# XuZhang1211/PVPUFormer

Hardware: AMD Instinct MI355X
Metric: 448x448 images/sec fwd+bwd, ViT-B VPUFormer (higher is better)
Workload: dtype bf16

## Files before the change

include/vpu_hip.h:

```cpp
#ifndef VPU_HIP_H
#define VPU_HIP_H
#include <stdint.h>

#ifdef __cplusplus
extern "C" {
#endif

#define VPU_BF16 0
#define VPU_F32 1

#define VPU_EPI_BIAS 1
#define VPU_EPI_PREACT 2
#define VPU_EPI_GELU 4
#define VPU_EPI_RELU 8
#define VPU_EPI_DGELU 16
#define VPU_EPI_DRELU 32
#define VPU_EPI_RESID 64
#define VPU_EPI_AFFINE 128
#define VPU_EPI_ACCUM 256
#define VPU_EPI_OUT_F32 512
#define VPU_EPI_SAVE_DGELU 1024
#define VPU_EPI_MULAUX 2048

typedef struct vpu_gemm_desc {
// ... 141 lines not shown
int vpu_click_keys_batched(const vpu_eval_obj* objs, int32_t n, uint8_t* err, int32_t* scratch, float* dist, int32_t Hm,
                           int32_t Wm, int32_t max_hw, void* stream);
typedef struct vpu_box_row {
    const float* prev;
    const uint8_t* gt;
    const uint8_t* valid;
    int32_t H, W, r0, r1, c0, c1, mirror, n_obj;
} vpu_box_row;
int vpu_box_prompts_batched(const vpu_box_row* rows, int32_t n_rows, const float* points, int32_t n_batch, int32_t S_h,
                            int32_t S_w, float pred_thresh, uint8_t* masks, int32_t* counts, int32_t* roots, int32_t* slots,
                            int32_t* table, int32_t kmax, int32_t* boxes, int32_t* flag, void* stream);
int vpu_cc_roots(const uint8_t* mask, int32_t* roots, int32_t B, int32_t H, int32_t W, void* stream);
int vpu_cc_table(const int32_t* roots, int32_t* slots, int32_t* table, int32_t kmax, int32_t B, int32_t H, int32_t W,
                 void* stream);

int vpu_disk_maps(const float* points, const int32_t* boxes, float* out, int32_t B, int32_t n, int32_t H, int32_t W,
                  float radius, void* stream);

int vpu_patch_im2col(const float* image4, const float* disks, void* cols, int32_t B, int32_t H, int32_t W, int32_t P,
                     int32_t win_tokens, int32_t dtype, void* stream);
int vpu_patch_im2col_prenorm(const float* image4, const float* disks, void* cols, int32_t B, int32_t H, int32_t W, int32_t P,
                             int32_t win_tokens, int32_t dtype, void* stream);
int vpu_patch_im2col_floor(const float* image4, const float* disks, void* cols, int32_t B, int32_t H, int32_t W, int32_t P,
                           int32_t wside, int32_t prenorm, int32_t dtype, void* stream);
int vpu_window_permute(const void* x, void* y, int32_t B, int32_t g, int32_t wg, int32_t C, int32_t dir, int32_t dtype,
                       void* stream);

int vpu_pixel_shuffle2(const void* in, void* out, const float* bias, int32_t B, int32_t h, int32_t w, int32_t C,
                       int32_t dir, int32_t dtype, void* stream);
int vpu_space_to_depth2_crop(const void* in, void* out, int32_t B, int32_t g, int32_t C, int32_t dir, int32_t dtype,
                             void* stream);
int vpu_pixel_shuffle2_gn_stats(const void* in, void* out, const float* bias, double* stats, int32_t B, int32_t h, int32_t w,
                                int32_t C, int32_t dtype, void* stream);
int vpu_groupnorm_apply(const void* x, const float* w, const float* b, void* y, float* mean, float* rstd, const double* stats,
                        int32_t B, int64_t HW, int32_t C, float eps, int32_t gelu, int32_t dtype, void* stream);
int vpu_pixel_unshuffle2_nblk(int32_t C);
int vpu_pixel_unshuffle2_sums(const void* in, void* out, float* part, int32_t B, int32_t h, int32_t w, int32_t C,
                              int32_t dtype, void* stream);
int vpu_groupnorm_nchunk(void);
int vpu_groupnorm_fwd(const void* x, const float* w, const float* b, void* y, float* mean, float* rstd, double* stats,
                      int32_t B, int64_t HW, int32_t C, float eps, int32_t gelu, int32_t dtype, void* stream);
int vpu_groupnorm_bwd(const void* dy, const void* x, const float* w, const float* b, const float* mean,
                      const float* rstd, void* dx, float* part, double* stats, int32_t B, int64_t HW, int32_t C,
                      int32_t gelu, int32_t dtype, void* stream);
int vpu_bilinear_cl_fwd(const void* in, int32_t ld_in, void* out, int32_t ld_out, int32_t B, int32_t h, int32_t w,
                        int32_t H, int32_t W, int32_t C, int32_t dtype, void* stream);
int vpu_bilinear_cl_bwd(const void* dout, int32_t ld_out, void* din, int32_t ld_in, int32_t B, int32_t h, int32_t w,
                        int32_t H, int32_t W, int32_t C, int32_t dtype, void* stream);
int vpu_upsum_relu(void* io, const void* const* z, const int32_t* h, const int32_t* w, int32_t n, int32_t B, int32_t H,
                   int32_t W, int32_t C, int32_t dtype, void* stream);
int vpu_head_grad_fused(const void* dfn, const void* y, const float* inv, const float* dout, const void* x, const float* w,
                        const float* mask, void* dx, float* part, float* part_b, int64_t rows, int64_t HW, int32_t C,
                        int32_t dtype, void* stream);
int vpu_gate_stats(const void* Q, const void* Kt, float* cg, int32_t* argq, float* sg, int32_t* argc, int32_t B,
                   int32_t nq, int32_t N, int32_t C, int32_t dtype, void* stream);
int vpu_gate_apply(const void* x, const float* cg, const float* sg, void* out, int32_t B, int32_t N, int32_t C,
                   int32_t dtype, void* stream);
int vpu_gate_bwd(const void* dout, const void* x, const float* cg, const int32_t* argq, const float* sg,
                 const int32_t* argc, void* dx, int32_t accum, void* dQ, void* dK, float* part, int32_t B, int32_t nq,
                 int32_t N, int32_t C, int32_t dtype, void* stream);
int vpu_gate_fwd_n(const void* const* Q, const void* const* K, const void* x, void* const* out, float* cg, int32_t* argq,
                   float* sg, int32_t* argc, int32_t n, int32_t B, int32_t nq, int32_t N, int32_t C, int32_t dtype, void* stream);
int vpu_gate_bwd_n(const void* const* dout, const void* x, const float* cg, const int32_t* argq, const float* sg,
                   const int32_t* argc, void* dx, int32_t accum, void* const* dQ, void* const* dK, float* part, int32_t n,
                   int32_t B, int32_t nq, int32_t N, int32_t C, int32_t dtype, void* stream);
int vpu_convseg_fwd(const void* x, const float* w, const float* bias, const float* mask, float* out, int64_t rows,
                    int64_t HW, int32_t C, int32_t dtype, void* stream);
int vpu_convseg_bwd_nblk(int64_t rows);
int vpu_convseg_bwd(const float* dout, const void* x, const float* w, const float* mask, void* dx, int32_t accum,
                    float* part, float* part_b, int64_t rows, int64_t HW, int32_t C, int32_t dtype, void* stream);

int vpu_upsample_ac_fwd(const float* in, float* out, int64_t planes, int32_t h, int32_t w, int32_t H, int32_t W,
                        void* stream);
int vpu_upsample_ac_bwd(const float* dout, float* din, int64_t planes, int32_t h, int32_t w, int32_t H, int32_t W,
                        void* stream);
int vpu_p2cl_fwd_bwd(const float* prob, const float* gt, const int32_t* slot_mask_idx, const float* override_masks,
                     float* loss_part, float* dprob, float grad_scale, int32_t B, int32_t S, int32_t H, int32_t W,
                     void* stream);
int vpu_p2cl_up_nband(int32_t h, int32_t w);
int vpu_p2cl_up_fwd_bwd(const float* sim_low, const float* gt, const int32_t* slot_mask_idx, const float* override_masks,
                        float* loss_part, float* dsim_low, float grad_scale, int32_t B, int32_t S, int32_t h, int32_t w,
                        int32_t H, int32_t W, void* stream);
int vpu_nfl_dice_scratch_doubles(int32_t B);
int vpu_nfl_dice_fwd_bwd(const float* logits, const float* gt, double* sums, float* out, float* dlogits, float w_nfl,
                         float w_dice, int32_t B, int64_t HW, void* stream);

int vpu_loss_finalize(const float* out, const float* part, int32_t B, int32_t npart, double inv_count, float w_nfl,
                      float w_dice, float w_pcl, float iter_weight, float* res, void* stream);

int vpu_adam_step(float* p, const float* g, float* m, float* v, void* shadow_bf16, int64_t n, float lr, float beta1,
                  float beta2, float eps, float weight_decay, int32_t step, float grad_scale, void* stream);
int vpu_adam_step_groups(float* p, const float* g, float* m, float* v, void* shadow_bf16, int64_t n,
                         const int64_t* seg_end, const float* seg_lr, const float* seg_wd, int32_t nseg, float beta1,
                         float beta2, float eps, int32_t decoupled_wd, int32_t step, float grad_scale, void* stream);
int vpu_adam_step_hyper(float* p, const float* g, float* m, float* v, void* shadow_bf16, int64_t n, const float* hyper,
                        const int64_t* seg_end, const float* seg_scale, const float* seg_wd, int32_t nseg, float beta1,
                        float beta2, float eps, float weight_decay, int32_t decoupled_wd, void* stream);


#ifdef __cplusplus
}
#endif
#endif
```

pvpuformer_amd/_lib.py:

```python
import ctypes as C
import os

_HERE = os.path.dirname(os.path.abspath(__file__))
LIB_PATH = os.path.join(_HERE, os.environ.get("VPU_LIB_FILE") or
                        ("libvpu_hip_diag.so" if os.environ.get("VPU_LIB_DIAG", "0") == "1" else "libvpu_hip.so"))

BF16, F32 = 0, 1

EPI_BIAS, EPI_PREACT, EPI_GELU, EPI_RELU, EPI_DGELU, EPI_DRELU = 1, 2, 4, 8, 16, 32
EPI_RESID, EPI_AFFINE, EPI_ACCUM, EPI_OUT_F32 = 64, 128, 256, 512
EPI_SAVE_DGELU, EPI_MULAUX = 1024, 2048


class GemmDesc(C.Structure):
    _fields_ = [
        ("A", C.c_void_p), ("B", C.c_void_p), ("C", C.c_void_p), ("bias", C.c_void_p), ("resid", C.c_void_p),
        ("aux", C.c_void_p), ("preact", C.c_void_p),
        ("M", C.c_int32), ("N", C.c_int32), ("K", C.c_int32),
        ("lda", C.c_int32), ("ldb", C.c_int32), ("ldc", C.c_int32), ("ldr", C.c_int32), ("ldaux", C.c_int32),
        ("batch", C.c_int32), ("inner", C.c_int32),
        ("sAo", C.c_int64), ("sAi", C.c_int64), ("sBo", C.c_int64), ("sBi", C.c_int64),
        ("sCo", C.c_int64), ("sCi", C.c_int64), ("sRo", C.c_int64), ("sRi", C.c_int64),
        ("transA", C.c_int32), ("transB", C.c_int32), ("dtype", C.c_int32), ("flags", C.c_int32),
        ("resid_period", C.c_int32),
# ... 44 lines not shown
    "vpu_l2norm_fwd": [_P, _P, _P, _L, _I, _I, _P],
    "vpu_l2norm_bwd": [_P, _P, _P, _P, _L, _I, _I, _P],
    "vpu_attn_fwd": [_P, _P, _P, _P, _P, _I, _I, _I, _I, _I, _I, _F, _P],
    "vpu_attn_bwd": [_P, _P, _P, _P, _P, _P, _P, _P, _P, _P, _I, _I, _I, _I, _I, _I, _I, _F, _P],
    "vpu_xattn_fwd": [_P, _P, _P, _P, _P, _I, _I, _I, _I, _I, _I, _I, _I, _F, _P],
    "vpu_xattn_bwd": [_P, _P, _P, _P, _P, _P, _P, _P, _P, _P, _I, _I, _I, _I, _I, _I, _I, _I, _I, _I, _F, _P],
    "vpu_xattn_fwd_split": [_P, _P, _P, _P, _P, _I, _I, _I, _I, _I, _I, _I, _I, _F, _I, _I, _P],
    "vpu_xattn_bwd_split": [_P, _P, _P, _P, _P, _P, _P, _P, _P, _P, _I, _I, _I, _I, _I, _I, _I, _I, _I, _I, _F, _I, _I, _P],
    "vpu_attn_combine": [_P, _P, _P, _P, _I, _I, _I, _I, _I, _I, _I, _P],
    "vpu_sum_groups": [_P, _P, _L, _I, _L, _I, _P],
    "vpu_add_bcast": [_P, _P, _P, _L, _L, _I, _P],
    "vpu_add4": [_P, _P, _P, _P, _P, _L, _I, _P],
    "vpu_cast2d": [_P, _I, _L, _P, _I, _L, _L, _I, _I, _P],
    "vpu_cast2d_batched": [C.POINTER(CastJob), _I, _P],
    "vpu_fanout_add": [_P, C.POINTER(C.c_void_p), C.POINTER(C.c_int32), _I, _L, _I, _P],
    "vpu_dropout_mask": [_P, _I, _F, C.c_uint64, _P, _P],
    "vpu_fill_f32": [_P, _F, _L, _P],
    "vpu_fill_ranges_f32": [_P, C.POINTER(C.c_int64), C.POINTER(C.c_int64), _I, _F, _P],
    "vpu_debug_spin": [_P, _I, _L, _P],
    "vpu_debug_gemm_times": [_P],
    "vpu_sigmoid_to_channel": [_P, _P, _I, _L, _I, _I, _P],
    "vpu_act_bwd": [_P, _L, _P, _L, _P, _L, _L, _I, _I, _I, _P],
    "vpu_pue_encode": [_P, _P, _P, _P, _P, _I, _I, _I, _I, _I, _I, _P],
    "vpu_cc_roots": [_P, _P, _I, _I, _I, _P],
    "vpu_cc_table": [_P, _P, _P, _I, _I, _I, _I, _P],
    "vpu_edt": [_P, _P, _P, _I, _I, _I, _I, _P],
    "vpu_chamfer5": [_P, _P, _P, _I, _I, _I, _I, _P],
    "vpu_pue_scribble_rows": [_P, _P, _P, _P, _I, _I, _I, _I, _I, _I, _P],
    "vpu_draw_polyline": [_P, _P, _I, _I, _I, _I, _P],
    "vpu_mask_bbox": [_P, _F, _P, _I, _P, _I, _I, _I, _P],
    "vpu_masked_argmax": [_P, _P, _P, _I, _I, _I, _P],
    "vpu_error_masks": [_P, _P, _P, _P, _I, _I, _P],
    "vpu_roi_resize_batched": [_P, _I, _P, _I, _I, _I, _I, _P],
    "vpu_roi_paste_batched": [_P, _I, _P, _I, _I, _F, _F, _I, _P],
    "vpu_click_keys_batched": [_P, _I, _P, _P, _P, _I, _I, _I, _P],
    "vpu_box_prompts_batched": [_P, _I, _P, _I, _I, _I, _F, _P, _P, _P, _P, _P, _I, _P, _P, _P],
    "vpu_disk_maps": [_P, _P, _P, _I, _I, _I, _I, _F, _P],
    "vpu_patch_im2col": [_P, _P, _P, _I, _I, _I, _I, _I, _I, _P],
    "vpu_patch_im2col_prenorm": [_P, _P, _P, _I, _I, _I, _I, _I, _I, _P],
    "vpu_patch_im2col_floor": [_P, _P, _P, _I, _I, _I, _I, _I, _I, _I, _P],
    "vpu_window_permute": [_P, _P, _I, _I, _I, _I, _I, _I, _P],
    "vpu_space_to_depth2_crop": [_P, _P, _I, _I, _I, _I, _I, _P],
    "vpu_pixel_shuffle2": [_P, _P, _P, _I, _I, _I, _I, _I, _I, _P],
    "vpu_pixel_shuffle2_gn_stats": [_P, _P, _P, _P, _I, _I, _I, _I, _I, _P],
    "vpu_groupnorm_apply": [_P, _P, _P, _P, _P, _P, _P, _I, _L, _I, _F, _I, _I, _P],
    "vpu_pixel_unshuffle2_nblk": [_I],
    "vpu_pixel_unshuffle2_sums": [_P, _P, _P, _I, _I, _I, _I, _I, _P],
    "vpu_groupnorm_nchunk": [],
    "vpu_groupnorm_fwd": [_P, _P, _P, _P, _P, _P, _P, _I, _L, _I, _F, _I, _I, _P],
    "vpu_groupnorm_bwd": [_P, _P, _P, _P, _P, _P, _P, _P, _P, _I, _L, _I, _I, _I, _P],
    "vpu_bilinear_cl_fwd": [_P, _I, _P, _I, _I, _I, _I, _I, _I, _I, _I, _P],
    "vpu_bilinear_cl_bwd": [_P, _I, _P, _I, _I, _I, _I, _I, _I, _I, _I, _P],
    "vpu_head_grad_fused": [_P, _P, _P, _P, _P, _P, _P, _P, _P, _P, _L, _L, _I, _I, _P],
    "vpu_upsum_relu": [_P, C.POINTER(C.c_void_p), C.POINTER(C.c_int32), C.POINTER(C.c_int32), _I, _I, _I, _I, _I, _I, _P],
    "vpu_gate_stats": [_P, _P, _P, _P, _P, _P, _I, _I, _I, _I, _I, _P],
    "vpu_gate_apply": [_P, _P, _P, _P, _I, _I, _I, _I, _P],
    "vpu_gate_bwd": [_P, _P, _P, _P, _P, _P, _P, _I, _P, _P, _P, _I, _I, _I, _I, _I, _P],
    "vpu_gate_fwd_n": [C.POINTER(C.c_void_p), C.POINTER(C.c_void_p), _P, C.POINTER(C.c_void_p), _P, _P, _P, _P, _I, _I, _I, _I, _I, _I, _P],
    "vpu_gate_bwd_n": [C.POINTER(C.c_void_p), _P, _P, _P, _P, _P, _P, _I, C.POINTER(C.c_void_p), C.POINTER(C.c_void_p), _P, _I, _I, _I,
                       _I, _I, _I, _P],
    "vpu_convseg_fwd": [_P, _P, _P, _P, _P, _L, _L, _I, _I, _P],
    "vpu_convseg_bwd_nblk": [_L],
    "vpu_convseg_bwd": [_P, _P, _P, _P, _P, _I, _P, _P, _L, _L, _I, _I, _P],
    "vpu_upsample_ac_fwd": [_P, _P, _L, _I, _I, _I, _I, _P],
    "vpu_upsample_ac_bwd": [_P, _P, _L, _I, _I, _I, _I, _P],
    "vpu_p2cl_fwd_bwd": [_P, _P, _P, _P, _P, _P, _F, _I, _I, _I, _I, _P],
    "vpu_p2cl_up_nband": [_I, _I],
    "vpu_p2cl_up_fwd_bwd": [_P, _P, _P, _P, _P, _P, _F, _I, _I, _I, _I, _I, _I, _P],
    "vpu_nfl_dice_scratch_doubles": [_I],
    "vpu_nfl_dice_fwd_bwd": [_P, _P, _P, _P, _P, _F, _F, _I, _L, _P],
    "vpu_loss_finalize": [_P, _P, _I, _I, C.c_double, _F, _F, _F, _F, _P, _P],
    "vpu_adam_step": [_P, _P, _P, _P, _P, _L, _F, _F, _F, _F, _F, _I, _F, _P],
    "vpu_adam_step_groups": [_P, _P, _P, _P, _P, _L, _P, _P, _P, _I, _F, _F, _F, _I, _I, _F, _P],
    "vpu_adam_step_hyper": [_P, _P, _P, _P, _P, _L, _P, _P, _P, _P, _I, _F, _F, _F, _F, _I, _P],
    "vpu_gemm_set_option": [C.c_char_p, _I],
    "vpu_gemm_get_option": [C.c_char_p, C.POINTER(C.c_int32)],
    "vpu_gemm_last_kernel": [],
    "vpu_attn_last_kernel": [],
    "vpu_attn_set_option": [C.c_char_p, _I],
    "vpu_gemm_grouped": [C.POINTER(GemmDesc), _I, _P],
    "vpu_last_error": [],
    "vpu_abi_version": [],
}
_RET = {"vpu_last_error": C.c_char_p, "vpu_gemm_last_kernel": C.c_char_p, "vpu_attn_last_kernel": C.c_char_p}

_lib = None


class VpuError(RuntimeError):
    pass


def load():
    global _lib
    if _lib is not None:
        return _lib
    if not os.path.exists(LIB_PATH):
        raise VpuError(f"{LIB_PATH} not found: build it with pvpuformer_amd/csrc/build.sh "
                       f"(or `python -c 'import __graft_entry__ as g; g.build()'`). There is no CPU fallback.")
    import torch
    lib = C.CDLL(LIB_PATH)
    for name, argtypes in SIGNATURES.items():
        fn = getattr(lib, name)
        fn.argtypes = argtypes
        fn.restype = _RET.get(name, C.c_int)
    _lib = lib
# ... 10 lines not shown
```

pvpuformer_amd/engine.py:

```python
import contextlib
import math
import os
from collections import OrderedDict
from types import SimpleNamespace

import numpy as np
import torch

from . import ops
from ._lib import (BF16, F32, EPI_BIAS, EPI_PREACT, EPI_GELU, EPI_RELU, EPI_DGELU, EPI_DRELU, EPI_RESID, EPI_AFFINE,
                   EPI_ACCUM, EPI_OUT_F32, EPI_SAVE_DGELU, EPI_MULAUX)


class Tape:
    __slots__ = ("fns", "out_grads", "done", "sim_low", "lane")

    def __init__(self):
        self.fns = []
        self.out_grads = [None, None, None]
        self.done = False
        self.sim_low = None
        self.lane = None

    def append(self, fn):
# ... 42 lines not shown
    pe[half + 1::2] = torch.cos(ph).t().unsqueeze(2).expand(-1, -1, width)
    return pe.reshape(d_model, height * width).t().contiguous()


def window_geometry(S, P):
    S, P = int(S), int(P)
    wg = 224 // P
    g = S // P if P > 0 else 0
    if P < 1 or wg < 1 or g < wg:
        raise ValueError(f"input side {S} with patch {P}: the token grid S // P = {g} must hold at least one "
                         f"{wg}-token window (S >= {wg * P})")
    nwin = g // wg
    if g % nwin:
        raise ValueError(f"input side {S} with patch {P}: the token grid g = S // P = {g} must split into nwin = g // {wg} = "
                         f"{nwin} equal windows per side (g % nwin == 0), as the reference's patchify requires")
    return g, nwin, g // nwin


def check_square(H, W):
    if H != W:
        raise ValueError(f"input {H}x{W}: only square inputs are supported (the reference's neck takes h = w = sqrt(HW))")


class Engine:
    def __init__(self, cfg, dtype="bf16", device="cuda"):
        self.cfg = dict(cfg)
        self.dt = BF16 if dtype in ("bf16", BF16) else F32
        self.td = torch.bfloat16 if self.dt == BF16 else torch.float32
        self.dev = torch.device(device)
        c = self.cfg
        self.D, self.P, self.img = c["embed_dim"], c["patch"], c["img"]
        self.g, _, self.wside = window_geometry(self.img, self.P)
        self.NT = self.g * self.g
        self.heads = c["num_heads"]
        self.depth = c["depth"]
        self.group = 6 if self.depth == 12 else self.depth // 4
        self.nmax = c["num_max_points"]
        self.E = 2 * self.img + 3
        self.Epad = _rup(self.E, 8)
        self.C = c["head_channels"]
        self.out_dims = tuple(c["out_dims"])
        self.names = None
        self.tape = Tape()
        self.last_tape = None
        self.params = []
        self.norm_radius = float(c.get("norm_radius", 5))
        self.training = False
        self.shadow_valid = False
        self._const_ready = False
        self.use_flash = True
        self.use_side = os.environ.get("VPU_WGRAD_STREAM", "0") == "1"
        self.side = None
        self.fuse_ln_pe = True
        self.group_wgrad = True
        self.ride_wgrad = True
        self.wgrad_fill = 0.8
        hid = self.D * c["mlp_ratio"]
        blk = sum(((n + 255) // 256) * ((k + 127) // 128) for n, k in ((3 * self.D, self.D), (self.D, self.D), (hid, self.D), (self.D, hid)))
        pk = os.environ.get("VPU_WGRAD_PACK", "")
        k3 = ops.gemm_get_option("k3")
        k4_default = (k3 & 8) != 0
        self.pack_wgrad = pk == "1" or (pk != "0" and (blk < 0.95 * 256 or k4_default))
        self.k3_wgrad = (k3 & 1) != 0
        self.k4_wgrad = (k3 & 8) != 0
        self.wgrad_round = 256 if (self.k4_wgrad or not self.k3_wgrad) else 512
        self.wgrad_tn = 256 if self.k4_wgrad else 128
        self.unify_wgrad = True
        self.lazy_zero = True
        self.xattn_split = max(1, int(os.environ.get("VPU_XATTN_SPLIT", "1")))
        self.neck_lanes = int(os.environ.get("VPU_NECK_LANES", "0"))
        self._tok_stream = None
        self._in_lanes = False
        self.dist_colsum = True
        self._pack_seen, self._pack_total = {}, {}
        self._pending_reports, self._reporting = [], False
        self.group_tiles = 256
        self.split_wgrad = True
        self._wq = []
        self._csq = []
        self._gq = []
        self._gq_out = set()
        self._frozen = set()
        self._token_rows = 0
        self.grad_ready_hook = None
        self.report_lag = max(1, int(os.environ.get("VPU_DIST_REPORT_LAG", "2")))

    def bind(self, named_params):
        self.names = OrderedDict()
        off = 0
        for n, p in named_params.items():
            self.names[n] = (off, tuple(p.shape), p.numel())
            off = _rup(off + p.numel(), 8)
        self.total = off
        self.flat = torch.zeros(off, device=self.dev, dtype=torch.float32)
        self.gflat = torch.zeros(off, device=self.dev, dtype=torch.float32)
        self.params = []
        for n, p in named_params.items():
            o, shape, numel = self.names[n]
            view = self.flat[o:o + numel].view(shape)
            view.copy_(p.data)
            p.data = view
            p.grad = self.gflat[o:o + numel].view(shape)
            self.params.append((p, o, shape, numel))
        self.shadow = torch.zeros(off, device=self.dev, dtype=torch.bfloat16) if self.dt == BF16 else None
        self._lazy = set()
        self._lazy_names, self._lazy_ranges = self._lazy_plan()
# ... 942 lines not shown
        B, H, W_, nq, o, tape = cx.B, cx.H, cx.W, cx.nq, self.out_dims, self.tape
        Cc, Hs = self.C, 4 * cx.g
        HW4 = Hs * Hs
        wf, ldf = self.W("head.fusion_conv.conv.weight"), 4 * Cc
        gf = self.G("head.fusion_conv.conv.weight")
        relu_done, ymask = [False], [[False] for _ in range(4)]
        ys, zs = [], []
        for i in range(4):
            f, s = feats[i]
            ys.append(self.linear(f, f"head.convs.{i}.conv.weight", f"head.convs.{i}.conv.bias", B * s * s, Cc, o[i],
                                  act="relu", pre_masked=ymask[i]))
        fused = Var(self._new(B * HW4, Cc))
        ops.gemm(ys[0].t, wf, fused.t, B * HW4, Cc, Cc, Cc, ldf, Cc, self.dt, flags=EPI_BIAS,
                 bias=self.Pm("head.fusion_conv.conv.bias"))
        for i in (1, 2, 3):
            s = feats[i][1]
            z = self._new(B * s * s, Cc)
            ops.gemm(ys[i].t, (wf[0], wf[1] + i * Cc), z, B * s * s, Cc, Cc, Cc, ldf, Cc, self.dt)
            zs.append((z, s, s))
        ops.upsum_relu(fused.t, zs, B, Hs, Hs, Cc, self.dt)
        if cx.training:
            def bwd_fusion():
                if fused.g is None:
                    return
                if relu_done[0]:
                    dt_ = fused.g
                else:
                    dt_ = self._new(B * HW4, Cc)
                    ops.act_bwd(fused.g, Cc, fused.t, Cc, dt_, Cc, B * HW4, Cc, 0, self.dt)
                self._wgrad(dt_, Cc, ys[0].t, Cc, gf, Cc, Cc, B * HW4, ldc=ldf, bias="head.fusion_conv.conv.bias")
                fuse_mask = self.dt == BF16
                mk = dict(flags=EPI_DRELU, ldaux=Cc) if fuse_mask else {}
                self._dgrad(dt_, Cc, wf, ldf, ys[0], B * HW4, Cc, Cc, **(dict(mk, aux=ys[0].t) if fuse_mask else {}))
                ymask[0][0] = fuse_mask
                for i in (1, 2, 3):
                    s = feats[i][1]
                    dz = self._new(B * s * s, Cc)
                    ops.bilinear_cl_bwd(dt_, Cc, dz, Cc, B, s, s, Hs, Hs, Cc, self.dt)
                    self._wgrad(dz, Cc, ys[i].t, Cc, (gf[0], gf[1] + i * Cc), Cc, Cc, B * s * s, ldc=ldf)
                    self._dgrad(dz, Cc, (wf[0], wf[1] + i * Cc), ldf, ys[i], B * s * s, Cc, Cc,
                                **(dict(mk, aux=ys[i].t) if fuse_mask else {}))
                    ymask[i][0] = fuse_mask
            self.tape.append(bwd_fusion)
        seg = self._new(B * HW4, dtype=torch.float32)
        ops.convseg_fwd(fused.t, self.Pm("head.conv_seg.weight"), self.Pm("head.conv_seg.bias"), drop_mask, seg,
                        B * HW4, HW4, Cc)
        dm = self.cfg["head_d_model"]
        query = self.mlp(q_out, "head.ffn_layer.lin1", "head.ffn_layer.lin2", B * nq, dm, 2 * dm, Cc, "relu")
        qn, fn = Var(torch.empty_like(query.t)), Var(torch.empty_like(fused.t))
        inv_q, inv_f = self._new(B * nq, dtype=torch.float32), self._new(B * HW4, dtype=torch.float32)
        ops.l2norm_fwd(query.t, qn.t, inv_q, B * nq, Cc)
        ops.l2norm_fwd(fused.t, fn.t, inv_f, B * HW4, Cc)
        sim = self._new(B, nq, HW4, dtype=torch.float32)
        ops.gemm(qn.t, fn.t, sim, nq, HW4, Cc, Cc, Cc, HW4, self.dt, flags=EPI_OUT_F32 | EPI_AFFINE, post_mul=0.5,
                 post_add=0.5, batch=B, inner=1, sA=(nq * Cc, 0), sB=(HW4 * Cc, 0), sC=(nq * HW4, 0))
        if cx.taps is not None:
            cx.taps["seg_lowres"] = seg.view(B, 1, Hs, Hs)
            cx.taps["sim_lowres"] = sim.view(B, nq, Hs, Hs)
            cx.taps["fused"] = fused.t
        inst = self._new(B, 1, H, W_, dtype=torch.float32)
        ops.upsample_ac_fwd(seg, inst, B, Hs, Hs, H, W_)
        aux = None
        self.sim_low = sim.view(B, nq, Hs, Hs)
        if materialize_aux:
            aux = self._new(B, nq, H, W_, dtype=torch.float32)
            ops.upsample_ac_fwd(sim, aux, B * nq, Hs, Hs, H, W_)
        tape.sim_low = self.sim_low
        if cx.training:
            def bwd_head():
                d_inst, d_aux, d_sim_low = tape.out_grads
                if d_aux is not None or d_sim_low is not None:
                    if d_sim_low is not None:
                        dsim = d_sim_low.view(B, nq, HW4)
                    else:
                        dsim = self._new(B, nq, HW4, dtype=torch.float32)
                        ops.upsample_ac_bwd(d_aux, dsim, B * nq, Hs, Hs, H, W_)
                    if self.dt == BF16:
                        dsim_t = self._new(B, nq, HW4)
                        ops.cast2d(dsim, HW4, dsim_t, HW4, B * nq, HW4)
                    else:
                        dsim_t = dsim
                    qn.g, fn.g = torch.empty_like(qn.t), torch.empty_like(fn.t)
                    ops.gemm(dsim_t, fn.t, qn.g, nq, Cc, HW4, HW4, Cc, Cc, self.dt, transB=True, alpha=0.5, batch=B,
                             inner=1, sA=(nq * HW4, 0), sB=(HW4 * Cc, 0), sC=(nq * Cc, 0))
                    ops.gemm(dsim_t, qn.t, fn.g, HW4, Cc, nq, HW4, Cc, Cc, self.dt, transA=True, transB=True, alpha=0.5,
                             batch=B, inner=1, sA=(nq * HW4, 0), sB=(nq * Cc, 0), sC=(HW4 * Cc, 0))
                    query.g = torch.empty_like(query.t)
                    ops.l2norm_bwd(qn.g, qn.t, inv_q, query.g, B * nq, Cc)
                    one_pass = d_inst is not None and self.dt == BF16 and Cc in (64, 128, 256, 512)
                    if not one_pass:
                        fused.g = torch.empty_like(fused.t)
                        ops.l2norm_bwd(fn.g, fn.t, inv_f, fused.g, B * HW4, Cc)
                if d_inst is not None:
                    dseg = self._new(B * HW4, dtype=torch.float32)
                    ops.upsample_ac_bwd(d_inst, dseg, B, Hs, Hs, H, W_)
                    nb = ops.convseg_bwd_nblk(B * HW4)
                    part, part_b = self._new(nb, Cc, dtype=torch.float32), self._new(nb, dtype=torch.float32)
                    if (d_aux is not None or d_sim_low is not None) and one_pass:
                        fused.g = torch.empty_like(fused.t)
                        ops.head_grad_fused(fn.g, fn.t, inv_f, dseg, fused.t, self.Pm("head.conv_seg.weight"), drop_mask,
                                            fused.g, part, part_b, B * HW4, HW4, Cc)
                    else:
                        accum = fused.g is not None
                        if not accum:
                            fused.g = torch.empty_like(fused.t)
                        self._writable(fused.g)
                        ops.convseg_bwd(dseg, fused.t, self.Pm("head.conv_seg.weight"), drop_mask, fused.g, int(accum) | 2, part,
                                        part_b, B * HW4, HW4, Cc)
                    relu_done[0] = True
                    self._csq.append((part, self.G("head.conv_seg.weight"), nb, Cc))
                    self._csq.append((part_b, self.G("head.conv_seg.bias"), nb, 1))
            self.tape.append(bwd_head)
        return inst, aux

    def _mark_ready(self, first_name, next_name):
        lo = self.names[first_name][0]
        hi = self.total if next_name is None else self.names[next_name][0]

        def marker():
            if self.ride_wgrad and self.group_wgrad and self.dt == BF16 and not self.use_side:
                self.flush_wgrads(0)
                if self.grad_ready_hook is not None:
                    for k in sorted({e[3] for e in self._wq if e[3] > 2048} - {self._token_rows}):
                        self.flush_wgrads(k)
                    self._pending_reports.append((lo, hi))
                    self._report_ready()
                    if len(self._pending_reports) > self.report_lag:
                        lo0, hi0 = self._pending_reports[0]
                        off_of = lambda t: t[1] if isinstance(t, tuple) else None
                        late = [e for e in self._wq
                                if any(off_of(t) is None or lo0 <= off_of(t) < hi0 for t in self._targets(e))]
                        if late:
                            self.flush_wgrads(entries=late)
                return
            self.flush_wgrads()
            if self.grad_ready_hook is not None:
                self._pending_reports.append((lo, hi))
                self._report_ready()
        self.tape.append(marker)
# ... 260 lines not shown
```

pvpuformer_amd/ops.py:

```python
import ctypes as C

import torch

from . import _lib
from ._lib import (BF16, F32, EPI_BIAS, EPI_PREACT, EPI_GELU, EPI_RELU, EPI_DGELU, EPI_DRELU, EPI_RESID, EPI_AFFINE,
                   EPI_ACCUM, EPI_OUT_F32, EPI_SAVE_DGELU, EPI_MULAUX, GemmDesc)

TORCH_DTYPE = {BF16: torch.bfloat16, F32: torch.float32}


def code_of(t):
    if isinstance(t, tuple):
        t = t[0]
    if t.dtype == torch.bfloat16:
        return BF16
    if t.dtype == torch.float32:
        return F32
    raise TypeError(f"unsupported dtype {t.dtype}")


_raw_stream = getattr(torch._C, "_cuda_getCurrentRawStream", None)
_cur_device = getattr(torch._C, "_cuda_getDevice", None)


# ... 462 lines not shown
    n = len(maps)
    zp = (C.c_void_p * 3)(*[ptr(m[0]) for m in maps])
    hs = (C.c_int32 * 3)(*[m[1] for m in maps])
    ws = (C.c_int32 * 3)(*[m[2] for m in maps])
    _lib.call("vpu_upsum_relu", ptr(io), zp, hs, ws, n, B, H, W, Cdim, dtype, _stream())


def gate_stats(Q, Kt, cg, argq, sg, argc, B, nq, N, Cdim):
    _lib.call("vpu_gate_stats", ptr(Q), ptr(Kt), ptr(cg), ptr(argq), ptr(sg), ptr(argc), B, nq, N, Cdim, code_of(Q),
              _stream())


def gate_apply(x, cg, sg, out, B, N, Cdim):
    _lib.call("vpu_gate_apply", ptr(x), ptr(cg), ptr(sg), ptr(out), B, N, Cdim, code_of(x), _stream())


def gate_bwd(dout, x, cg, argq, sg, argc, dx, accum, dQ, dK, part, B, nq, N, Cdim):
    _lib.call("vpu_gate_bwd", ptr(dout), ptr(x), ptr(cg), ptr(argq), ptr(sg), ptr(argc), ptr(dx), int(accum), ptr(dQ),
              ptr(dK), ptr(part), B, nq, N, Cdim, code_of(x), _stream())


def _ptr_array(ts):
    return (C.c_void_p * len(ts))(*[ptr(t) for t in ts])


def gate_fwd_n(Qs, Ks, x, outs, cg, argq, sg, argc, B, nq, N, Cdim):
    _lib.call("vpu_gate_fwd_n", _ptr_array(Qs), _ptr_array(Ks), ptr(x), _ptr_array(outs), ptr(cg), ptr(argq), ptr(sg), ptr(argc),
              len(Qs), B, nq, N, Cdim, code_of(x), _stream())


def gate_bwd_n(douts, x, cg, argq, sg, argc, dx, accum, dQs, dKs, part, B, nq, N, Cdim):
    _lib.call("vpu_gate_bwd_n", _ptr_array(douts), ptr(x), ptr(cg), ptr(argq), ptr(sg), ptr(argc), ptr(dx), int(accum),
              _ptr_array(dQs), _ptr_array(dKs), ptr(part), len(douts), B, nq, N, Cdim, code_of(x), _stream())


def convseg_fwd(x, w, bias, mask, out, rows, HW, Cdim):
    _lib.call("vpu_convseg_fwd", ptr(x), ptr(w), ptr(bias), ptr(mask), ptr(out), rows, HW, Cdim, code_of(x), _stream())


def convseg_bwd_nblk(rows):
    return _lib.load().vpu_convseg_bwd_nblk(rows)


def convseg_bwd(dout, x, w, mask, dx, accum, part, part_b, rows, HW, Cdim):
    _lib.call("vpu_convseg_bwd", ptr(dout), ptr(x), ptr(w), ptr(mask), ptr(dx), int(accum), ptr(part), ptr(part_b),
              rows, HW, Cdim, code_of(x), _stream())


def head_grad_fused(dfn, y, inv, dout, x, w, mask, dx, part, part_b, rows, HW, Cdim):
    _lib.call("vpu_head_grad_fused", ptr(dfn), ptr(y), ptr(inv), ptr(dout), ptr(x), ptr(w), ptr(mask), ptr(dx), ptr(part),
              ptr(part_b), rows, HW, Cdim, code_of(x), _stream())


def upsample_ac_fwd(inp, out, planes, h, w, H, W):
    _lib.call("vpu_upsample_ac_fwd", ptr(inp), ptr(out), planes, h, w, H, W, _stream())


def upsample_ac_bwd(dout, din, planes, h, w, H, W):
    _lib.call("vpu_upsample_ac_bwd", ptr(dout), ptr(din), planes, h, w, H, W, _stream())


def p2cl_fwd_bwd(prob, gt, slot_idx, override, loss_part, dprob, grad_scale, B, S, H, W):
    _lib.call("vpu_p2cl_fwd_bwd", ptr(prob), ptr(gt), ptr(slot_idx), ptr(override), ptr(loss_part), ptr(dprob),
              grad_scale, B, S, H, W, _stream())


def p2cl_up_fwd_bwd(sim_low, gt, slot_idx, override, loss_part, dsim_low, grad_scale, B, S, h, w, H, W):
    nband = _lib.load().vpu_p2cl_up_nband(h, w)
    bands = torch.empty(B * S, nband, device=sim_low.device, dtype=torch.float32)
    _lib.call("vpu_p2cl_up_fwd_bwd", ptr(sim_low), ptr(gt), ptr(slot_idx), ptr(override), ptr(bands), ptr(dsim_low),
              grad_scale, B, S, h, w, H, W, _stream())
    if loss_part is None:
        return bands
    torch.sum(bands, dim=1, out=loss_part.view(B * S))
    return loss_part


def nfl_dice_fwd_bwd(logits, gt, sums, out, dlogits, w_nfl, w_dice, B, HW):
    if sums is None:
        sums = torch.empty(_lib.load().vpu_nfl_dice_scratch_doubles(B), device=logits.device, dtype=torch.float64)
    _lib.call("vpu_nfl_dice_fwd_bwd", ptr(logits), ptr(gt), ptr(sums), ptr(out), ptr(dlogits), w_nfl, w_dice, B, HW,
              _stream())


def loss_finalize(out, part, B, npart, inv_count, w_nfl, w_dice, w_pcl, iter_weight, res):
    _lib.call("vpu_loss_finalize", ptr(out), ptr(part), B, npart, float(inv_count), w_nfl, w_dice, w_pcl, iter_weight,
              ptr(res), _stream())


def adam_step_groups(p, g, m, v, shadow, n, seg_end, seg_lr, seg_wd, nseg, b1, b2, eps, decoupled, step, grad_scale=1.0):
    _lib.call("vpu_adam_step_groups", ptr(p), ptr(g), ptr(m), ptr(v), ptr(shadow), n, ptr(seg_end), ptr(seg_lr),
              ptr(seg_wd), nseg, b1, b2, eps, int(decoupled), step, grad_scale, _stream())


def adam_step_hyper(p, g, m, v, shadow, n, hyper, seg_end, seg_scale, seg_wd, nseg, b1, b2, eps, wd, decoupled):
    _lib.call("vpu_adam_step_hyper", ptr(p), ptr(g), ptr(m), ptr(v), ptr(shadow), n, ptr(hyper), ptr(seg_end),
              ptr(seg_scale), ptr(seg_wd), nseg, b1, b2, eps, wd, int(decoupled), _stream())


def adam_step(p, g, m, v, shadow, n, lr, b1, b2, eps, wd, step, grad_scale=1.0):
    _lib.call("vpu_adam_step", ptr(p), ptr(g), ptr(m), ptr(v), ptr(shadow), n, lr, b1, b2, eps, wd, step, grad_scale,
              _stream())
```

Baseline: 1013.

## Add dedicated skinny-GEMM kernels for query-pixel similarity forward and backward

Replaces the generic batched GEMM for the query-by-pixel similarity map, which has a small query count, with a specialized MFMA kernel. The kernel keeps the normalized queries in LDS and streams the pixel features with register double-buffering. The backward path fuses the fp32-to-bf16 cast of dsim into a single kernel that computes both dfn and per-chunk dqn partials, followed by a small reduce kernel. This removes the cast pass and one GEMM launch. The cost is extra hand-written code with shape restrictions (nq<=64, C in a fixed set, HW%16==0), with fallback to the generic GEMM otherwise.

```diff
diff --git a/include/vpu_hip.h b/include/vpu_hip.h
--- a/include/vpu_hip.h
+++ b/include/vpu_hip.h
@@ -217,6 +217,11 @@
 int vpu_head_grad_fused(const void* dfn, const void* y, const float* inv, const float* dout, const void* x, const float* w,
                         const float* mask, void* dx, float* part, float* part_b, int64_t rows, int64_t HW, int32_t C,
                         int32_t dtype, void* stream);
+int vpu_sim_fwd(const void* qn, const void* fn, float* sim, int32_t B, int32_t nq, int64_t HW, int32_t C, int32_t dtype,
+                void* stream);
+int vpu_sim_bwd_nchunk(int32_t B, int64_t HW);
+int vpu_sim_bwd(const float* dsim, const void* qn, const void* fn, void* dqn, void* dfn, float* part, int32_t B, int32_t nq,
+                int64_t HW, int32_t C, int32_t dtype, void* stream);
 int vpu_gate_stats(const void* Q, const void* Kt, float* cg, int32_t* argq, float* sg, int32_t* argc, int32_t B,
                    int32_t nq, int32_t N, int32_t C, int32_t dtype, void* stream);
 int vpu_gate_apply(const void* x, const float* cg, const float* sg, void* out, int32_t B, int32_t N, int32_t C,
diff --git a/pvpuformer_amd/_lib.py b/pvpuformer_amd/_lib.py
--- a/pvpuformer_amd/_lib.py
+++ b/pvpuformer_amd/_lib.py
@@ -120,6 +120,9 @@
     "vpu_bilinear_cl_fwd": [_P, _I, _P, _I, _I, _I, _I, _I, _I, _I, _I, _P],
     "vpu_bilinear_cl_bwd": [_P, _I, _P, _I, _I, _I, _I, _I, _I, _I, _I, _P],
     "vpu_head_grad_fused": [_P, _P, _P, _P, _P, _P, _P, _P, _P, _P, _L, _L, _I, _I, _P],
+    "vpu_sim_fwd": [_P, _P, _P, _I, _I, _L, _I, _I, _P],
+    "vpu_sim_bwd_nchunk": [_I, _L],
+    "vpu_sim_bwd": [_P, _P, _P, _P, _P, _P, _I, _I, _L, _I, _I, _P],
     "vpu_upsum_relu": [_P, C.POINTER(C.c_void_p), C.POINTER(C.c_int32), C.POINTER(C.c_int32), _I, _I, _I, _I, _I, _I, _P],
     "vpu_gate_stats": [_P, _P, _P, _P, _P, _P, _I, _I, _I, _I, _I, _P],
     "vpu_gate_apply": [_P, _P, _P, _P, _I, _I, _I, _I, _P],
diff --git a/pvpuformer_amd/csrc/headsim.hip b/pvpuformer_amd/csrc/headsim.hip
--- /dev/null
+++ b/pvpuformer_amd/csrc/headsim.hip
@@ -0,0 +1,300 @@
+#include <stdio.h>
+#include <stdlib.h>
+#include "vpu_common.h"
+#include "../../include/vpu_hip.h"
+
+#define ST reinterpret_cast<hipStream_t>(stream)
+
+namespace {
+
+typedef __attribute__((address_space(3))) s16x4_t* lds_s16x4_ptr;
+
+__device__ __forceinline__ f32x4_t mfma16(const bf16x8_t& a, const bf16x8_t& b, const f32x4_t& c) {
+    return __builtin_amdgcn_mfma_f32_16x16x32_bf16(a, b, c, 0, 0, 0);
+}
+template <typename Off> __device__ __forceinline__ bf16x8_t frag_tr(const char* lds, int k0, int lane, Off off) {
+    const int g = lane >> 4, q = (lane & 15) >> 2, p = lane & 3;
+    const s16x4_t lo = __builtin_amdgcn_ds_read_tr16_b64_v4i16((lds_s16x4_ptr)(lds + off(k0 + 8 * g + q) + 8 * p));
+    const s16x4_t hi = __builtin_amdgcn_ds_read_tr16_b64_v4i16((lds_s16x4_ptr)(lds + off(k0 + 8 * g + 4 + q) + 8 * p));
+    s16x8_t v;
+    v[0] = lo[0]; v[1] = lo[1]; v[2] = lo[2]; v[3] = lo[3];
+    v[4] = hi[0]; v[5] = hi[1]; v[6] = hi[2]; v[7] = hi[3];
+    return __builtin_bit_cast(bf16x8_t, v);
+}
+
+template <int C>
+__global__ __launch_bounds__(256) void sim_fwd_kernel(const bf16_t* __restrict__ qn, const bf16_t* __restrict__ fn,
+                                                      float* __restrict__ sim, int nq, int HW, int per) {
+    constexpr int CPR = C / 8, KS = C / 32, SW = (CPR - 1) & 7;
+    __shared__ __attribute__((aligned(16))) char l_q[64 * C * 2];
+    const int tid = threadIdx.x, lane = tid & 63, wave = tid >> 6, b = blockIdx.y;
+    const int g = lane >> 4, r16 = lane & 15;
+    for (int i = tid; i < 64 * CPR; i += 256) {
+        const int q = i / CPR, ch = i % CPR;
+        uint4 v = make_uint4(0, 0, 0, 0);
+        if (q < nq) v = *reinterpret_cast<const uint4*>(qn + ((int64_t)b * nq + q) * C + ch * 8);
+        *reinterpret_cast<uint4*>(l_q + q * (C * 2) + ((ch ^ (q & SW)) << 4)) = v;
+    }
+    __syncthreads();
+    const int nunit = (HW + 63) / 64;
+    const int u0 = blockIdx.x * per, u1 = u0 + per < nunit ? u0 + per : nunit;
+    const bf16_t* fb = fn + (int64_t)b * HW * C;
+    float* sb = sim + (int64_t)b * nq * HW;
+    auto fetch = [&](int u, uint4 (&a)[KS]) {
+        const int p = u * 64 + wave * 16 + r16;
+        const bf16_t* row = fb + (int64_t)(p < HW ? p : HW - 1) * C + g * 8;
+#pragma unroll
+        for (int ks = 0; ks < KS; ++ks) a[ks] = *reinterpret_cast<const uint4*>(row + ks * 32);
+    };
+    auto products = [&](int u, const uint4 (&a)[KS]) {
+        const int p0 = u * 64 + wave * 16;
+        f32x4_t acc[4];
+#pragma unroll
+        for (int qt = 0; qt < 4; ++qt) acc[qt] = f32x4_t{0.f, 0.f, 0.f, 0.f};
+#pragma unroll
+        for (int ks = 0; ks < KS; ++ks) {
+            const bf16x8_t af = __builtin_bit_cast(bf16x8_t, a[ks]);
+#pragma unroll
+            for (int qt = 0; qt < 4; ++qt) {
+                const int q = 16 * qt + r16;
+                const uint4 v = *reinterpret_cast<const uint4*>(l_q + q * (C * 2) + (((ks * 4 + g) ^ (q & SW)) << 4));
+                acc[qt] = mfma16(af, __builtin_bit_cast(bf16x8_t, v), acc[qt]);
+            }
+        }
+        if (p0 < HW) {
+#pragma unroll
+            for (int qt = 0; qt < 4; ++qt) {
+                const int q = 16 * qt + r16;
+                if (q < nq) {
+                    const f32x4_t r = acc[qt];
+                    *reinterpret_cast<float4*>(sb + (int64_t)q * HW + p0 + 4 * g) =
+                        make_float4(0.5f * r[0] + 0.5f, 0.5f * r[1] + 0.5f, 0.5f * r[2] + 0.5f, 0.5f * r[3] + 0.5f);
+                }
+            }
+        }
+    };
+    uint4 ra[KS], rb[KS];
+    const int ul = u1 - 1;
+    fetch(u0 < ul ? u0 : ul, ra);
+    for (int u = u0; u < u1; u += 2) {
+        fetch(u + 1 < ul ? u + 1 : ul, rb);
+        products(u, ra);
+        fetch(u + 2 < ul ? u + 2 : ul, ra);
+        if (u + 1 < u1) products(u + 1, rb);
+    }
+}
+
+constexpr int DS_LD = 80;
+
+template <int T> __device__ __forceinline__ int fng_col(int t, int m) {
+    return T >= 2 ? 32 * (t >> 1) + 8 * (m >> 2) + 4 * (t & 1) + (m & 3) : m;
+}
+
+template <int C>
+__global__ __launch_bounds__(256, C <= 256 ? 2 : 1) void sim_bwd_kernel(const float* __restrict__ dsim, const bf16_t* __restrict__ qn,
+                                                      const bf16_t* __restrict__ fn, bf16_t* __restrict__ dfn,
+                                                      float* __restrict__ part, int nq, int HW) {
+    constexpr int CPR = C / 8, CW = C / 4, T = CW / 16, NF = 32 * CPR / 256, FM = (C / 16 - 1) & 7;
+    __shared__ __attribute__((aligned(16))) char l_fn[32 * C * 2];
+    __shared__ __attribute__((aligned(16))) char l_ds[64 * DS_LD];
+    const int tid = threadIdx.x, lane = tid & 63, wave = tid >> 6, b = blockIdx.y;
+    const int g = lane >> 4, r16 = lane & 15, wbase = wave * CW;
+    const int nchunk = gridDim.x, ntile = (HW + 31) / 32;
+    const bf16_t* fb = fn + (int64_t)b * HW * C;
+    const float* db = dsim + (int64_t)b * nq * HW;
+    bf16_t* gb = dfn + (int64_t)b * HW * C;
+    auto fsw = [](int row) { return ((row & 3) | (((row >> 3) & 1) << 2)) & FM; };
+
+    bf16x8_t qa[T][2];
+#pragma unroll
+    for (int t = 0; t < T; ++t)
+#pragma unroll
+        for (int ks = 0; ks < 2; ++ks)
+#pragma unroll
+            for (int j = 0; j < 8; ++j) {
+                const int q = ks * 32 + 8 * g + j;
+                const bf16_t v = qn[((int64_t)b * nq + (q < nq ? q : nq - 1)) * C + wbase + fng_col<T>(t, r16)];
+                qa[t][ks][j] = q < nq ? v : (bf16_t)0.f;
+            }
+
+    uint4 rf[NF];
+    float4 rd[2];
+    auto fetch = [&](int t) {
+        const int p0 = t * 32;
+#pragma unroll
+        for (int i = 0; i < NF; ++i) {
+            const int idx = tid + i * 256, row = idx / CPR, ch = idx % CPR, p = p0 + row;
+            rf[i] = *reinterpret_cast<const uint4*>(fb + (int64_t)(p < HW ? p : HW - 1) * C + ch * 8);
+        }
+#pragma unroll
+        for (int i = 0; i < 2; ++i) {
+            const int idx = tid + i * 256, q = idx >> 3, p = p0 + (idx & 7) * 4;
+            rd[i] = *reinterpret_cast<const float4*>(db + (int64_t)(q < nq ? q : nq - 1) * HW + (p < HW ? p : HW - 4));
+        }
+    };
+    f32x4_t accq[4][T];
+#pragma unroll
+    for (int i = 0; i < 4; ++i)
+#pragma unroll
+        for (int t = 0; t < T; ++t) accq[i][t] = f32x4_t{0.f, 0.f, 0.f, 0.f};
+
+    int t = blockIdx.x;
+    fetch(t);
+    for (; t < ntile; t += nchunk) {
+        const int p0 = t * 32;
+#pragma unroll
+        for (int i = 0; i < NF; ++i) {
+            const int idx = tid + i * 256, row = idx / CPR, ch = idx % CPR;
+            *reinterpret_cast<uint4*>(l_fn + row * (C * 2) + (((ch >> 1) ^ fsw(row)) << 5) + ((ch & 1) << 4)) =
+                p0 + row < HW ? rf[i] : make_uint4(0, 0, 0, 0);
+        }
+#pragma unroll
+        for (int i = 0; i < 2; ++i) {
+            const int idx = tid + i * 256, q = idx >> 3, x = (idx & 7) * 4;
+            typedef bf16_t bf16x4_t __attribute__((ext_vector_type(4)));
+            const bool live = q < nq && p0 + x < HW;
+            bf16x4_t v;
+            v[0] = (bf16_t)(live ? rd[i].x : 0.f); v[1] = (bf16_t)(live ? rd[i].y : 0.f);
+            v[2] = (bf16_t)(live ? rd[i].z : 0.f); v[3] = (bf16_t)(live ? rd[i].w : 0.f);
+            *reinterpret_cast<bf16x4_t*>(l_ds + q * DS_LD + x * 2) = v;
+        }
+        __syncthreads();
+        fetch(t + nchunk < ntile ? t + nchunk : ntile - 1);
+
+        bf16x8_t da[4];
+#pragma unroll
+        for (int i = 0; i < 4; ++i)
+            da[i] = __builtin_bit_cast(bf16x8_t, *reinterpret_cast<const uint4*>(l_ds + (16 * i + r16) * DS_LD + g * 16));
+#pragma unroll
+        for (int tt = 0; tt < T; ++tt) {
+            const int slot = (wbase + 16 * tt) >> 4;
+            const bf16x8_t bf = frag_tr(l_fn, 0, lane, [&](int row) { return row * (C * 2) + ((slot ^ fsw(row)) << 5); });
+#pragma unroll
+            for (int i = 0; i < 4; ++i) accq[i][tt] = mfma16(da[i], bf, accq[i][tt]);
+        }
+        f32x4_t accf[T][2];
+#pragma unroll
+        for (int tt = 0; tt < T; ++tt) accf[tt][0] = accf[tt][1] = f32x4_t{0.f, 0.f, 0.f, 0.f};
+#pragma unroll
+        for (int ks = 0; ks < 2; ++ks)
+#pragma unroll
+            for (int nt = 0; nt < 2; ++nt) {
+                const bf16x8_t bd = frag_tr(l_ds, ks * 32, lane, [&](int row) { return row * DS_LD + nt * 32; });
+#pragma unroll
+                for (int tt = 0; tt < T; ++tt) accf[tt][nt] = mfma16(qa[tt][ks], bd, accf[tt][nt]);
+            }
+#pragma unroll
+        for (int nt = 0; nt < 2; ++nt) {
+            const int p = p0 + 16 * nt + r16;
+            if (p < HW) {
+                bf16_t* row = gb + (int64_t)p * C + wbase;
+                if constexpr (T >= 2) {
+#pragma unroll
+                    for (int u = 0; u < T / 2; ++u) {
+                        bf16x8_t o;
+#pragma unroll
+                        for (int r = 0; r < 4; ++r) {
+                            o[r] = (bf16_t)(0.5f * accf[2 * u][nt][r]);
+                            o[4 + r] = (bf16_t)(0.5f * accf[2 * u + 1][nt][r]);
+                        }
+                        *reinterpret_cast<bf16x8_t*>(row + 32 * u + 8 * g) = o;
+                    }
+                } else {
+                    typedef bf16_t bf16x4_t __attribute__((ext_vector_type(4)));
+                    bf16x4_t o;
+#pragma unroll
+                    for (int r = 0; r < 4; ++r) o[r] = (bf16_t)(0.5f * accf[0][nt][r]);
+                    *reinterpret_cast<bf16x4_t*>(row + 4 * g) = o;
+                }
+            }
+        }
+        __syncthreads();
+    }
+    float* pw = part + ((int64_t)b * nchunk + blockIdx.x) * nq * C;
+#pragma unroll
+    for (int i = 0; i < 4; ++i)
+#pragma unroll
+        for (int tt = 0; tt < T; ++tt)
+#pragma unroll
+            for (int r = 0; r < 4; ++r) {
+                const int q = 16 * i + 4 * g + r;
+                if (q < nq) pw[(int64_t)q * C + wbase + 16 * tt + r16] = accq[i][tt][r];
+            }
+}
+
+__global__ __launch_bounds__(256) void sim_bwd_reduce_kernel(const float* __restrict__ part, bf16_t* __restrict__ dqn,
+                                                             int nchunk, int nqc, int total4) {
+    const int i = blockIdx.x * 256 + threadIdx.x;
+    if (i >= total4) return;
+    const int per = nqc / 4, b = i / per, e = (i % per) * 4;
+    const float* p = part + (int64_t)b * nchunk * nqc + e;
+    float4 s = make_float4(0.f, 0.f, 0.f, 0.f);
+#pragma unroll 8
+    for (int k = 0; k < nchunk; ++k) {
+        const float4 v = *reinterpret_cast<const float4*>(p + (int64_t)k * nqc);
+        s.x += v.x; s.y += v.y; s.z += v.z; s.w += v.w;
+    }
+    typedef bf16_t bf16x4_t __attribute__((ext_vector_type(4)));
+    bf16x4_t o;
+    o[0] = (bf16_t)(0.5f * s.x); o[1] = (bf16_t)(0.5f * s.y); o[2] = (bf16_t)(0.5f * s.z); o[3] = (bf16_t)(0.5f * s.w);
+    *reinterpret_cast<bf16x4_t*>(dqn + (int64_t)b * nqc + e) = o;
+}
+
+bool sim_args_ok(const char* who, int B, int nq, int64_t HW, int C, int dtype) {
+    if (dtype != VPU_BF16 || B < 1 || B > 65535 || nq < 1 || nq > 64 || (C != 64 && C != 128 && C != 256 && C != 512) ||
+        HW < 16 || HW % 16 || HW > (1 << 30)) {
+        static thread_local char msg[160];
+        snprintf(msg, sizeof msg, "%s: bf16 only, 1 <= nq <= 64, C in {64, 128, 256, 512}, HW %% 16 == 0, B <= 65535", who);
+        vpu_set_error(msg);
+        return false;
+    }
+    return true;
+}
+
+int sim_bwd_nchunk(int B, int64_t HW) {
+    const int64_t ntile = (HW + 31) / 32;
+    int64_t want = 512 / (B < 1 ? 1 : B);
+    if (want < 1) want = 1;
+    const int64_t per = (ntile + want - 1) / want;
+    return (int)((ntile + per - 1) / per);
+}
+
+}
+
+#define SIM_DISPATCH_C(C, ...)                  \
+    switch (C) {                                \
+        case 64: { constexpr int CC = 64; __VA_ARGS__ } break;   \
+        case 128: { constexpr int CC = 128; __VA_ARGS__ } break; \
+        case 256: { constexpr int CC = 256; __VA_ARGS__ } break; \
+        default: { constexpr int CC = 512; __VA_ARGS__ } break;  \
+    }
+
+extern "C" int vpu_sim_fwd(const void* qn, const void* fn, float* sim, int32_t B, int32_t nq, int64_t HW, int32_t C,
+                           int32_t dtype, void* stream) {
+    vpu_clear_stale_error();
+    if (!sim_args_ok("sim_fwd", B, nq, HW, C, dtype)) return VPU_ERR_ARG;
+    if (!qn || !fn || !sim) { vpu_set_error("sim_fwd: null operand"); return VPU_ERR_ARG; }
+    const int64_t nunit = (HW + 63) / 64;
+    int64_t want = 512 / B;
+    if (want < 1) want = 1;
+    const int per = (int)((nunit + want - 1) / want);
+    const dim3 grid((unsigned)((nunit + per - 1) / per), (unsigned)B);
+    SIM_DISPATCH_C(C, sim_fwd_kernel<CC><<<grid, 256, 0, ST>>>((const bf16_t*)qn, (const bf16_t*)fn, sim, nq, (int)HW, per);)
+    return vpu_check_launch("vpu_sim_fwd");
+}
+
+extern "C" int vpu_sim_bwd_nchunk(int32_t B, int64_t HW) { return sim_bwd_nchunk(B, HW); }
+
+extern "C" int vpu_sim_bwd(const float* dsim, const void* qn, const void* fn, void* dqn, void* dfn, float* part, int32_t B,
+                           int32_t nq, int64_t HW, int32_t C, int32_t dtype, void* stream) {
+    vpu_clear_stale_error();
+    if (!sim_args_ok("sim_bwd", B, nq, HW, C, dtype)) return VPU_ERR_ARG;
+    if (!dsim || !qn || !fn || !dqn || !dfn || !part) { vpu_set_error("sim_bwd: null operand"); return VPU_ERR_ARG; }
+    const int nchunk = sim_bwd_nchunk(B, HW);
+    const dim3 grid((unsigned)nchunk, (unsigned)B);
+    SIM_DISPATCH_C(C, sim_bwd_kernel<CC><<<grid, 256, 0, ST>>>(dsim, (const bf16_t*)qn, (const bf16_t*)fn, (bf16_t*)dfn, part,
+                                                               nq, (int)HW);)
+    const int total4 = B * nq * C / 4;
+    sim_bwd_reduce_kernel<<<(total4 + 255) / 256, 256, 0, ST>>>(part, (bf16_t*)dqn, nchunk, nq * C, total4);
+    return vpu_check_launch("vpu_sim_bwd");
+}
diff --git a/pvpuformer_amd/engine.py b/pvpuformer_amd/engine.py
--- a/pvpuformer_amd/engine.py
+++ b/pvpuformer_amd/engine.py
@@ -118,6 +118,7 @@
         self.use_side = os.environ.get("VPU_WGRAD_STREAM", "0") == "1"
         self.side = None
         self.fuse_ln_pe = True
+        self.head_stream = True
         self.group_wgrad = True
         self.ride_wgrad = True
         self.wgrad_fill = 0.8
@@ -1166,8 +1167,12 @@
         ops.l2norm_fwd(query.t, qn.t, inv_q, B * nq, Cc)
         ops.l2norm_fwd(fused.t, fn.t, inv_f, B * HW4, Cc)
         sim = self._new(B, nq, HW4, dtype=torch.float32)
-        ops.gemm(qn.t, fn.t, sim, nq, HW4, Cc, Cc, Cc, HW4, self.dt, flags=EPI_OUT_F32 | EPI_AFFINE, post_mul=0.5,
-                 post_add=0.5, batch=B, inner=1, sA=(nq * Cc, 0), sB=(HW4 * Cc, 0), sC=(nq * HW4, 0))
+        stream_sim = self.head_stream and ops.sim_shape_ok(self.dt, nq, HW4, Cc)
+        if stream_sim:
+            ops.sim_fwd(qn.t, fn.t, sim, B, nq, HW4, Cc)
+        else:
+            ops.gemm(qn.t, fn.t, sim, nq, HW4, Cc, Cc, Cc, HW4, self.dt, flags=EPI_OUT_F32 | EPI_AFFINE, post_mul=0.5,
+                     post_add=0.5, batch=B, inner=1, sA=(nq * Cc, 0), sB=(HW4 * Cc, 0), sC=(nq * HW4, 0))
         if cx.taps is not None:
             cx.taps["seg_lowres"] = seg.view(B, 1, Hs, Hs)
             cx.taps["sim_lowres"] = sim.view(B, nq, Hs, Hs)
@@ -1189,16 +1194,20 @@
                     else:
                         dsim = self._new(B, nq, HW4, dtype=torch.float32)
                         ops.upsample_ac_bwd(d_aux, dsim, B * nq, Hs, Hs, H, W_)
-                    if self.dt == BF16:
-                        dsim_t = self._new(B, nq, HW4)
-                        ops.cast2d(dsim, HW4, dsim_t, HW4, B * nq, HW4)
+                    qn.g, fn.g = torch.empty_like(qn.t), torch.empty_like(fn.t)
+                    if stream_sim:
+                        part = self._new(B, ops.sim_bwd_nchunk(B, HW4), nq, Cc, dtype=torch.float32)
+                        ops.sim_bwd(dsim, qn.t, fn.t, qn.g, fn.g, part, B, nq, HW4, Cc)
                     else:
-                        dsim_t = dsim
-                    qn.g, fn.g = torch.empty_like(qn.t), torch.empty_like(fn.t)
-                    ops.gemm(dsim_t, fn.t, qn.g, nq, Cc, HW4, HW4, Cc, Cc, self.dt, transB=True, alpha=0.5, batch=B,
-                             inner=1, sA=(nq * HW4, 0), sB=(HW4 * Cc, 0), sC=(nq * Cc, 0))
-                    ops.gemm(dsim_t, qn.t, fn.g, HW4, Cc, nq, HW4, Cc, Cc, self.dt, transA=True, transB=True, alpha=0.5,
-                             batch=B, inner=1, sA=(nq * HW4, 0), sB=(nq * Cc, 0), sC=(HW4 * Cc, 0))
+                        if self.dt == BF16:
+                            dsim_t = self._new(B, nq, HW4)
+                            ops.cast2d(dsim, HW4, dsim_t, HW4, B * nq, HW4)
+                        else:
+                            dsim_t = dsim
+                        ops.gemm(dsim_t, fn.t, qn.g, nq, Cc, HW4, HW4, Cc, Cc, self.dt, transB=True, alpha=0.5, batch=B,
+                                 inner=1, sA=(nq * HW4, 0), sB=(HW4 * Cc, 0), sC=(nq * Cc, 0))
+                        ops.gemm(dsim_t, qn.t, fn.g, HW4, Cc, nq, HW4, Cc, Cc, self.dt, transA=True, transB=True, alpha=0.5,
+                                 batch=B, inner=1, sA=(nq * HW4, 0), sB=(nq * Cc, 0), sC=(HW4 * Cc, 0))
                     query.g = torch.empty_like(query.t)
                     ops.l2norm_bwd(qn.g, qn.t, inv_q, query.g, B * nq, Cc)
                     one_pass = d_inst is not None and self.dt == BF16 and Cc in (64, 128, 256, 512)
diff --git a/pvpuformer_amd/ops.py b/pvpuformer_amd/ops.py
--- a/pvpuformer_amd/ops.py
+++ b/pvpuformer_amd/ops.py
@@ -538,6 +538,23 @@
               ptr(part_b), rows, HW, Cdim, code_of(x), _stream())
 
 
+def sim_fwd(qn, fn, sim, B, nq, HW, Cdim):
+    _lib.call("vpu_sim_fwd", ptr(qn), ptr(fn), ptr(sim), B, nq, HW, Cdim, code_of(fn), _stream())
+
+
+def sim_shape_ok(dtype, nq, HW, Cdim):
+    return dtype == BF16 and 1 <= nq <= 64 and Cdim in (64, 128, 256, 512) and HW >= 16 and HW % 16 == 0
+
+
+def sim_bwd_nchunk(B, HW):
+    return _lib.load().vpu_sim_bwd_nchunk(B, HW)
+
+
+def sim_bwd(dsim, qn, fn, dqn, dfn, part, B, nq, HW, Cdim):
+    _lib.call("vpu_sim_bwd", ptr(dsim), ptr(qn), ptr(fn), ptr(dqn), ptr(dfn), ptr(part), B, nq, HW, Cdim, code_of(fn),
+              _stream())
+
+
 def upsample_ac_fwd(inp, out, planes, h, w, H, W):
     _lib.call("vpu_upsample_ac_fwd", ptr(inp), ptr(out), planes, h, w, H, W, _stream())
 
```

After: 1020, median of 6. No clear change (+0.7%).
